# akanazawa/human_dynamics

Measured on NVIDIA H100. Metric: frames/sec (ResNet->f_movie->SMPL LBS), higher is better.
Workload: dtype f32 (wgmma 3x fp16 head/remainder split, fp32 two-level accumulate)

## Files before the change

### human_dynamics_b200/csrc/conv_tc.cu

```cuda
#include <cuda.h>
#include <cuda_fp16.h>
#include <cstdlib>
#include "conv_common.cuh"
#include "tc_ptx.cuh"

namespace hd {
namespace {

constexpr int BM = 128;
constexpr int A_TILE_BYTES = BM * 128;
constexpr int BOX_BYTES = 64 * 128;
constexpr int W_PROD = 8;
constexpr int STAGE_OUT = 1, STAGE_PAIR = 2;

using namespace ptx;

template <bool SPLIT, bool HALF, bool ASPLIT, int BN, bool RES = false, bool SHORT = false>
struct Cfg {
  static_assert(BN == 64 || (BN == 128 && HALF && ASPLIT), "128-wide N tiles: pre-split fp16 path only");
  static_assert(!RES || ASPLIT, "residual by TMA: pre-split fp16 path only");
  static_assert(!SHORT || (BN == 64 && HALF && ASPLIT), "two CTAs per SM: 64-wide pre-split fp16 tiles only");
  static constexpr int CTAS = SHORT ? 2 : 1;
  static constexpr int PROD_THREADS = BN == 128 || SHORT ? 128 : 256;
  static constexpr int NUM_THREADS = 256 + PROD_THREADS;
  static constexpr int ROW_STEP = PROD_THREADS / 8;
  static constexpr int ROWS = BM / ROW_STEP;
  static constexpr int PROD_REGS = SHORT ? 32 : BN == 128 ? 40 : 104, CONS_REGS = SHORT ? 104 : BN == 128 ? 232 : 152;
  static_assert(CTAS * (256 * CONS_REGS + PROD_THREADS * PROD_REGS) <= 65536, "setmaxnreg split beyond the register file");
  static constexpr int NACC = BN / 2;
  static constexpr int STAGES = SHORT ? 1 : BN == 128 ? (RES ? 2 : 3) : (RES ? 3 : 4);
  static constexpr int BKE = HALF ? 64 : 32;
  static constexpr int B_TILE_BYTES = BN * 128;
  static constexpr int B_OFFSET = (SPLIT ? 2 : 1) * A_TILE_BYTES;
  static constexpr int STAGE_BYTES = (SPLIT ? 2 : 1) * (A_TILE_BYTES + B_TILE_BYTES);
  static constexpr int RES_OFFSET = STAGES * STAGE_BYTES;
  static constexpr int RES_SLOT_BYTES = RES || SHORT ? 64 * BN * 4 : 0;
  static constexpr int STG_OFFSET = SHORT ? RES_OFFSET : RES_OFFSET + 2 * RES_SLOT_BYTES;
  static constexpr int STG_BYTES = ASPLIT ? 2 * BOX_BYTES : 0;
  static_assert(!SHORT || STG_BYTES == RES_SLOT_BYTES, "SHORT: the staging buffer is the residual slot");
  static constexpr int BAR_OFFSET = SHORT ? RES_OFFSET + 2 * RES_SLOT_BYTES : STG_OFFSET + 2 * STG_BYTES;
  static constexpr int SMEM_BYTES = BAR_OFFSET + 128 + 1024;
  static_assert(SMEM_BYTES <= 232448, "dynamic shared memory beyond the 227 KB a CTA can opt into");
  static_assert(CTAS * (SMEM_BYTES + 1024) <= 233472, "CTAS CTAs (and the 1 KB each reserves) beyond an SM's 228 KB");
  static constexpr int PF = HALF ? 2 : 3;
  static constexpr int V = HALF ? 2 : 1;
};

template <int R>
struct RowState {
  int n[R], iy[R], ix[R];
};

template <bool SPLIT, int PCH, bool HALF, bool GATHER, bool ASPLIT, int BN, bool RES, bool SHORT>
__global__ void __launch_bounds__((Cfg<SPLIT, HALF, ASPLIT, BN, RES, SHORT>::NUM_THREADS), (Cfg<SPLIT, HALF, ASPLIT, BN, RES, SHORT>::CTAS))
conv_gemm_tc_kernel(const ConvParams p, const __grid_constant__ CUtensorMap tmap_hi, const __grid_constant__ CUtensorMap tmap_lo,
                    const __grid_constant__ CUtensorMap tmap_res, const __grid_constant__ CUtensorMap tmap_out,
                    const __grid_constant__ CUtensorMap tmap_out_hi, const __grid_constant__ CUtensorMap tmap_out_lo, const int stage) {
  using C = Cfg<SPLIT, HALF, ASPLIT, BN, RES, SHORT>;
  constexpr bool MEM_STAMPS = BN == 128 || SHORT;
  constexpr int BKE = C::BKE, PF = C::PF, V = C::V, STAGES = C::STAGES, R = C::ROWS, RS = C::ROW_STEP, NA = C::NACC;
  extern __shared__ uint8_t smem_raw[];
  const uint32_t smem_base = (smem_u32(smem_raw) + 1023u) & ~1023u;
  uint8_t *smem = smem_raw + (smem_base - smem_u32(smem_raw));
  const uint32_t bar_base = smem_base + C::BAR_OFFSET;
  auto full_bar = [&](int s) { return bar_base + 8u * s; };
  auto empty_bar = [&](int s) { return bar_base + 8u * (STAGES + s); };
  auto res_bar = [&](int g) { return bar_base + 8u * (2 * STAGES + g); };

  const int warp = threadIdx.x >> 5, lane = threadIdx.x & 31;
  const int num_k = (GATHER ? p.K_pad : p.K) / BKE;
  const int tiles_n = (p.Cout + BN - 1) / BN;
  const int num_tiles = ((p.M + BM - 1) / BM) * tiles_n;
  const int my_tiles = (num_tiles - (int)blockIdx.x + (int)gridDim.x - 1) / (int)gridDim.x;

  if (threadIdx.x == 0) {
    for (int s = 0; s < STAGES; ++s) {
      mbar_init(full_bar(s), ASPLIT ? C::PROD_THREADS + 1 : 9);
      mbar_init(empty_bar(s), 8);
    }
    if (RES) for (int g = 0; g < 2; ++g) mbar_init(res_bar(g), 1);
    asm volatile("fence.mbarrier_init.release.cluster;" ::: "memory");
  }
  __syncthreads();

  if (warp >= W_PROD) {
    asm volatile("setmaxnreg.dec.sync.aligned.u32 %0;" ::"n"(C::PROD_REGS));
    const int t = threadIdx.x - W_PROD * 32;
    const int j = t & 7;
    const int rb = t >> 3;
    const uint32_t sw_off = (uint32_t)((j ^ (rb & 7)) << 4);
    const bool prof = p.dbg != nullptr && blockIdx.x == 0 && t == 0;
    long long t_wait = 0, t_start = prof && !MEM_STAMPS ? clock64() : 0;
    if (MEM_STAMPS && prof) { p.dbg[0] = clock64(); p.dbg[1] = 0; }
    auto wait_empty = [&](int s, uint32_t ph) {
      if (MEM_STAMPS && prof) p.dbg[1] -= clock64();
      const long long tw0 = !MEM_STAMPS && prof ? clock64() : 0;
      mbar_wait(empty_bar(s), ph ^ 1u);
      if (!MEM_STAMPS && prof) t_wait += clock64() - tw0;
      if (MEM_STAMPS && prof) p.dbg[1] += clock64();
    };
    const int total = my_tiles * num_k;
    auto load_b = [&](int s, int ti, int kc) {
      if (t != 0) return;
      const int n0 = (((int)blockIdx.x + ti * (int)gridDim.x) % tiles_n) * BN;
      const uint32_t b_hi = smem_base + s * C::STAGE_BYTES + C::B_OFFSET;
      const int boxes = (BN == 128 && n0 + 64 < p.Cout) ? 2 : 1;
      mbar_arrive_expect_tx(full_bar(s), (SPLIT ? 2 : 1) * boxes * BOX_BYTES);
      for (int b = 0; b < boxes; ++b) {
        tma_load_2d(b_hi + b * BOX_BYTES, &tmap_hi, full_bar(s), kc * BKE, n0 + 64 * b);
        if (SPLIT) tma_load_2d(b_hi + C::B_TILE_BYTES + b * BOX_BYTES, &tmap_lo, full_bar(s), kc * BKE, n0 + 64 * b);
      }
    };

    auto enter_tile = [&](int ti, RowState<R> &rs) {
      const int tile = (int)blockIdx.x + ti * (int)gridDim.x;
      const int m0 = (tile / tiles_n) * BM;
      const int hw = p.Ho * p.Wo;
#pragma unroll
      for (int i = 0; i < R; ++i) {
        const int m = m0 + rb + RS * i;
        if (m < p.M) {
          const int n = m / hw;
          const int r = m - n * hw;
          const int oy = r / p.Wo, ox = r - oy * p.Wo;
          rs.n[i] = n; rs.iy[i] = oy * p.stride - p.pad_t; rs.ix[i] = ox * p.stride - p.pad_l;
        } else {
          rs.n[i] = -1; rs.iy[i] = 0; rs.ix[i] = 0;
        }
      }
    };
    if constexpr (ASPLIT) {
      const __half *ihi = reinterpret_cast<const __half *>(p.in_hi);
      const __half *ilo = reinterpret_cast<const __half *>(p.in_lo);
      if (SHORT || (!p.planes && p.KH * p.KW <= 32 && (long long)p.n_img * p.H * p.W * p.in_ld < (1ll << 31))) {
        const uint32_t off0 = (uint32_t)rb * 128u + sw_off;
        int base[R];
        uint32_t mask[R];
        int kc = 0, ti = 0, tap = 0, ci0 = 0, kx = 0, ky = 0, tap_off = 0;
        for (int q = 0; q < total; ++q) {
          if (kc == 0) {
            const int tile = (int)blockIdx.x + ti * (int)gridDim.x;
            const int m0 = (tile / tiles_n) * BM + rb;
            const int hw = p.Ho * p.Wo;
#pragma unroll
            for (int i = 0; i < R; ++i) {
              const int m = m0 + RS * i;
              uint32_t mk = 0;
              int b = 0;
              if (m < p.M) {
                const int n = m / hw;
                const int r = m - n * hw;
                const int oy = r / p.Wo, ox = r - oy * p.Wo;
                const int iy0 = oy * p.stride - p.pad_t, ix0 = ox * p.stride - p.pad_l;
                b = ((n * p.H + iy0) * p.W + ix0) * p.in_ld + j * 8;
                int t = 0;
                for (int yy = 0; yy < p.KH; ++yy)
                  for (int xx = 0; xx < p.KW; ++xx, ++t)
                    if ((unsigned)(iy0 + yy) < (unsigned)p.H && (unsigned)(ix0 + xx) < (unsigned)p.W) mk |= 1u << t;
              }
              base[i] = SHORT && !(mk & 1u) ? -1 : b;
              mask[i] = mk;
            }
            tap = 0; ci0 = 0; kx = 0; ky = 0; tap_off = 0;
          }
          const int s = q % STAGES;
          const uint32_t ph = (uint32_t)(q / STAGES) & 1u;
          wait_empty(s, ph);
          load_b(s, ti, kc);
          const uint32_t a_hi = smem_base + s * C::STAGE_BYTES + off0;
          const int eo = SHORT ? ci0 : tap_off + ci0;
#pragma unroll
          for (int i = 0; i < R; ++i) {
            const bool ok = SHORT ? base[i] >= 0 : (mask[i] >> tap) & 1u;
            const int e = ok ? base[i] + eo : 0;
            cp_async16(a_hi + i * RS * 128, ihi + e, ok ? 16u : 0u);
            if (SPLIT) cp_async16(a_hi + A_TILE_BYTES + i * RS * 128, ilo + e, ok ? 16u : 0u);
          }
          asm volatile("cp.async.mbarrier.arrive.noinc.shared::cta.b64 [%0];" ::"r"(full_bar(s)) : "memory");
          ci0 += BKE;
          if (ci0 == p.Cin) {
            ci0 = 0; ++tap;
            if (++kx == p.KW) { kx = 0; ++ky; }
            tap_off = (ky * p.W + kx) * p.in_ld;
          }
          if (++kc == num_k) { kc = 0; ++ti; }
        }
      } else if (!SHORT && p.planes && (long long)p.n_img * p.H * p.W * p.in_ld < (1ll << 31)) {
        const uint32_t off0 = (uint32_t)rb * 128u + sw_off;
        const int jt = j >> 2;
        const int row_step = 2 * p.W * (int)p.in_ld;
        int base[R];
        int kc = 0, ti = 0;
        for (int q = 0; q < total; ++q) {
          if (kc == 0) {
            const int tile = (int)blockIdx.x + ti * (int)gridDim.x;
            const int m0 = (tile / tiles_n) * BM + rb;
            const int hw = p.Ho * p.Wo;
#pragma unroll
            for (int i = 0; i < R; ++i) {
              const int m = m0 + RS * i;
              int b = -1;
              if (m < p.M) {
                const int n = m / hw;
                const int r = m - n * hw;
                const int oy = r / p.Wo, ox = r - oy * p.Wo;
                b = ((n * p.H + oy * p.stride + jt) * p.W + ox * p.stride) * (int)p.in_ld + (j & 3) * 8;
              }
              base[i] = b;
            }
          }
          const int s = q % STAGES;
          const uint32_t ph = (uint32_t)(q / STAGES) & 1u;
          wait_empty(s, ph);
          load_b(s, ti, kc);
          const uint32_t a_hi = smem_base + s * C::STAGE_BYTES + off0;
          const bool tap_ok = 2 * kc + jt < 7;
          const int eo = kc * row_step;
#pragma unroll
          for (int i = 0; i < R; ++i) {
            const bool ok = tap_ok && base[i] >= 0;
            const int e = ok ? base[i] + eo : 0;
            cp_async16_ca(a_hi + i * RS * 128, ihi + e, ok ? 16u : 0u);
            if (SPLIT) cp_async16_ca(a_hi + A_TILE_BYTES + i * RS * 128, ilo + e, ok ? 16u : 0u);
          }
          asm volatile("cp.async.mbarrier.arrive.noinc.shared::cta.b64 [%0];" ::"r"(full_bar(s)) : "memory");
          if (++kc == num_k) { kc = 0; ++ti; }
        }
      } else if (!SHORT) {
      RowState<R> rs;
      int kc = 0, ti = 0;
      for (int q = 0; q < total; ++q) {
        if (kc == 0) enter_tile(ti, rs);
        const int s = q % STAGES;
        const uint32_t ph = (uint32_t)(q / STAGES) & 1u;
        wait_empty(s, ph);
        load_b(s, ti, kc);
        const int kb = kc * BKE;
        const int tap = p.planes ? 2 * kc + (j >> 2) : kb / p.Cin;
        const int ci = p.planes ? (j & 3) * 8 : kb - tap * p.Cin + j * 8;
        const int ky = tap / p.KW, kx = tap - ky * p.KW;
        const bool tap_ok = !p.planes || tap < 7;
        const uint32_t a_hi = smem_base + s * C::STAGE_BYTES, a_lo = a_hi + A_TILE_BYTES;
#pragma unroll
        for (int i = 0; i < R; ++i) {
          const int iy = rs.iy[i] + ky, ix = rs.ix[i] + kx;
          const bool ok = tap_ok && rs.n[i] >= 0 && iy >= 0 && iy < p.H && ix >= 0 && ix < p.W;
          const size_t e = ok ? ((size_t)((size_t)rs.n[i] * p.H + iy) * p.W + ix) * p.in_ld + ci : 0;
          const uint32_t off = (uint32_t)(rb + RS * i) * 128u + sw_off;
          if (p.planes) {
            cp_async16_ca(a_hi + off, ihi + e, ok ? 16u : 0u);
            if (SPLIT) cp_async16_ca(a_lo + off, ilo + e, ok ? 16u : 0u);
          } else {
            cp_async16(a_hi + off, ihi + e, ok ? 16u : 0u);
            if (SPLIT) cp_async16(a_lo + off, ilo + e, ok ? 16u : 0u);
          }
        }
        asm volatile("cp.async.mbarrier.arrive.noinc.shared::cta.b64 [%0];" ::"r"(full_bar(s)) : "memory");
        if (++kc == num_k) { kc = 0; ++ti; }
      }
      }
      cp_async_commit();
      cp_async_wait<0>();
      if (prof) { p.dbg[0] = clock64() - (MEM_STAMPS ? p.dbg[0] : t_start); if (!MEM_STAMPS) p.dbg[1] = t_wait; }
    } else {
    RowState<R> pf_rs, st_rs;
    float4 ring[PF][4 * V];
    uint32_t vmask[PF];
    int pf_kc = 0, pf_ti = 0;
    auto prefetch = [&](float4 *dst, uint32_t &vm) {
      if (pf_kc == 0) enter_tile(pf_ti, pf_rs);
      if (GATHER) {
        const int seg = p.KW * p.Cin, segp = (seg + 7) & ~7;
        const int g8 = (pf_kc * BKE + j * (4 * V)) / 8;
        const int gpr = segp >> 3;
        const int ky = g8 / gpr, r0 = (g8 - ky * gpr) * 8;
// ... 18 lines not shown
        if (++pf_kc == num_k) { pf_kc = 0; ++pf_ti; }
        return;
      }
      const int kb = pf_kc * BKE;
      const int tap = kb / p.Cin, ci = kb - tap * p.Cin + j * (4 * V);
      const int ky = tap / p.KW, kx = tap - ky * p.KW;
      vm = 0;
#pragma unroll
      for (int i = 0; i < 4; ++i) {
        const int iy = pf_rs.iy[i] + ky, ix = pf_rs.ix[i] + kx;
        const bool ok = pf_rs.n[i] >= 0 && (unsigned)iy < (unsigned)p.H && (unsigned)ix < (unsigned)p.W;
        if (ok) {
          const float4 *src = reinterpret_cast<const float4 *>(p.in + ((size_t)((size_t)pf_rs.n[i] * p.H + iy) * p.W + ix) * p.in_ld + ci);
#pragma unroll
          for (int v = 0; v < V; ++v) dst[i * V + v] = __ldg(src + v);
          vm |= 1u << i;
        } else {
#pragma unroll
          for (int v = 0; v < V; ++v) dst[i * V + v] = make_float4(0.f, 0.f, 0.f, 0.f);
        }
      }
      if (++pf_kc == num_k) { pf_kc = 0; ++pf_ti; }
    };
    int st_kc = 0, st_ti = 0;
    auto consume = [&](int q, float4 *cur, uint32_t vm) {
      if (st_kc == 0) enter_tile(st_ti, st_rs);
      const int s = q % STAGES;
      const uint32_t ph = (uint32_t)(q / STAGES) & 1u;
      long long tw0 = prof ? clock64() : 0;
      mbar_wait(empty_bar(s), ph ^ 1u);
      if (prof) t_wait += clock64() - tw0;
      load_b(s, st_ti, st_kc);
      uint8_t *a_hi = smem + s * C::STAGE_BYTES;
      uint8_t *a_lo = a_hi + A_TILE_BYTES;
      const int pci = p.pre_scale ? (st_kc * BKE) % p.Cin + j * (4 * V) : 0;
#pragma unroll
      for (int i = 0; i < 4; ++i) {
        float xs[4 * V];
#pragma unroll
        for (int v = 0; v < V; ++v) {
          const float4 x = cur[i * V + v];
          xs[4 * v] = x.x; xs[4 * v + 1] = x.y; xs[4 * v + 2] = x.z; xs[4 * v + 3] = x.w;
        }
        if (p.pre_scale && (vm & (1u << i))) {
          const size_t po = (size_t)(p.pre_img_stride != 0 ? st_rs.n[i] : 0) * p.pre_img_stride + pci;
#pragma unroll
          for (int v = 0; v < V; ++v) {
            const float4 sc = __ldg(reinterpret_cast<const float4 *>(p.pre_scale + po) + v);
            const float4 sh = __ldg(reinterpret_cast<const float4 *>(p.pre_shift + po) + v);
            xs[4 * v] = xs[4 * v] * sc.x + sh.x; xs[4 * v + 1] = xs[4 * v + 1] * sc.y + sh.y;
            xs[4 * v + 2] = xs[4 * v + 2] * sc.z + sh.z; xs[4 * v + 3] = xs[4 * v + 3] * sc.w + sh.w;
          }
          if (p.pre_relu) {
#pragma unroll
            for (int e = 0; e < 4 * V; ++e) xs[e] = fmaxf(xs[e], 0.f);
          }
        }
        uint32_t h[4], l[4];
        if (!HALF) {
#pragma unroll
          for (int e = 0; e < 4; ++e) {
            const float hf = rn_tf32(xs[e]);
            h[e] = __float_as_uint(hf);
            l[e] = __float_as_uint(rn_tf32(xs[e] - hf));
          }
        } else {
#pragma unroll
// ... 39 lines not shown
    for (int i = 0; i < NA; ++i) {
      acc[i] = 0.f;
      if constexpr (SPLIT) accx[i] = 0.f;
    }
    uint8_t *res_sm = smem + C::RES_OFFSET + wg * C::RES_SLOT_BYTES;
    const bool res_issuer = RES && (threadIdx.x & 127) == 0;
    const bool stg_issuer = ASPLIT && (threadIdx.x & 127) == 0;
    auto load_res = [&](int ti) {
      const int tile = (int)blockIdx.x + ti * (int)gridDim.x;
      const int r0 = (tile / tiles_n) * BM + 64 * wg, c0 = (tile % tiles_n) * BN;
      const int cols = p.Cout - c0 < BN ? p.Cout - c0 : BN;
      const int boxes = r0 < p.M ? (cols + 31) / 32 : 0;
      const uint32_t slot = smem_base + C::RES_OFFSET + wg * C::RES_SLOT_BYTES;
      mbar_arrive_expect_tx(res_bar(wg), boxes * (64 * 128));
      for (int b = 0; b < boxes; ++b) tma_load_2d(slot + b * (64 * 128), &tmap_res, res_bar(wg), c0 + 32 * b, r0);
    };
    if (res_issuer && my_tiles > 0) load_res(0);
    int q = 0;
    for (int ti = 0; ti < my_tiles; ++ti) {
      if (!SHORT) {
#pragma unroll
        for (int i = 0; i < NA; ++i) sums[i] = 0.f;
      }
      for (int kc = 0; kc < num_k; ++kc, ++q) {
        const int s = q % STAGES;
        const uint32_t ph = (uint32_t)(q / STAGES) & 1u;
        const bool group_start = (kc % PCH) == 0;
        if (MEM_STAMPS && prof) p.dbg[3] -= clock64();
        const long long tw0 = !MEM_STAMPS && prof ? clock64() : 0;
        mbar_wait(full_bar(s), ph);
        if (!MEM_STAMPS && prof) t_wait += clock64() - tw0;
        if (MEM_STAMPS && prof) p.dbg[3] += clock64();
        if (ASPLIT) asm volatile("fence.proxy.async.shared::cta;" ::: "memory");
        const uint32_t a_hi = smem_base + s * C::STAGE_BYTES + wg * (64 * 128);
        const uint32_t a_lo = a_hi + A_TILE_BYTES;
        const uint32_t b_hi = smem_base + s * C::STAGE_BYTES + C::B_OFFSET;
        const uint32_t b_lo = b_hi + C::B_TILE_BYTES;
        const uint64_t da_hi = make_smem_desc(a_hi), da_lo = make_smem_desc(a_lo);
        const uint64_t db_hi = make_smem_desc(b_hi), db_lo = make_smem_desc(b_lo);
        fence_regs(acc);
        if constexpr (SPLIT) fence_regs(accx);
        wgmma_fence();
#pragma unroll
        for (int k = 0; k < 4; ++k) {
          const uint64_t adv = (uint64_t)((k * 32) >> 4);
          if constexpr (BN == 128) {
            if constexpr (SPLIT) {
              wgmma_m64n128k16_f16(accx, da_lo + adv, db_hi + adv, (kc | k) != 0);
              wgmma_m64n128k16_f16(accx, da_hi + adv, db_lo + adv, 1u);
            }
            wgmma_m64n128k16_f16(acc, da_hi + adv, db_hi + adv, !(group_start && k == 0));
          } else if constexpr (HALF) {
            if constexpr (SPLIT) {
              wgmma_m64n64k16_f16(accx, da_lo + adv, db_hi + adv, (kc | k) != 0);
              wgmma_m64n64k16_f16(accx, da_hi + adv, db_lo + adv, 1u);
            }
            wgmma_m64n64k16_f16(acc, da_hi + adv, db_hi + adv, !(group_start && k == 0));
          } else {
            if constexpr (SPLIT) {
              wgmma_m64n64k8_tf32(accx, da_lo + adv, db_hi + adv, (kc | k) != 0);
              wgmma_m64n64k8_tf32(accx, da_hi + adv, db_lo + adv, 1u);
            }
            wgmma_m64n64k8_tf32(acc, da_hi + adv, db_hi + adv, !(group_start && k == 0));
          }
        }
        wgmma_commit();
        wgmma_wait<0>();
        fence_regs(acc);
        if constexpr (SPLIT) fence_regs(accx);
        __syncwarp();
        if (lane == 0) mbar_arrive(empty_bar(s));
        if (!SHORT && ((kc % PCH) == PCH - 1 || kc == num_k - 1)) {
#pragma unroll
          for (int i = 0; i < NA; ++i) sums[i] += acc[i];
        }
      }
      if (SHORT) {
#pragma unroll
        for (int i = 0; i < NA; ++i) acc[i] = __fadd_rn(0.f, acc[i]);
      }
      if constexpr (SPLIT) {
#pragma unroll
        for (int i = 0; i < NA; ++i) sums[i] += accx[i] * (HALF ? (1.0f / 2048.0f) : 1.0f);
      }
      if (prof) p.dbg[4] -= clock64();
      const int tile = (int)blockIdx.x + ti * (int)gridDim.x;
      const int m0 = (tile / tiles_n) * BM, n0 = (tile % tiles_n) * BN;
      if (RES && prof) p.dbg[5] -= clock64();
      if (RES) mbar_wait(res_bar(wg), (uint32_t)ti & 1u);
      if (RES && prof) p.dbg[5] += clock64();
      auto row_geom = [&](int m, int &n_img, int &oy, int &ox) {
        n_img = 0; oy = 0; ox = 0;
        if (p.out_sub || (!RES && p.res && !(p.res_stride == 1 && p.res_H == p.Ho && p.res_W == p.Wo))) {
          n_img = m / hw;
          const int r = m - n_img * hw;
          oy = r / p.Wo; ox = r - oy * p.Wo;
        }
      };
      auto res_row = [&](int m, int n_img, int oy, int ox) -> const float * {
        if (RES || !p.res) return nullptr;
        const size_t rr = (p.res_stride == 1 && p.res_H == p.Ho && p.res_W == p.Wo)
                              ? (size_t)m
                              : ((size_t)n_img * p.res_H + (size_t)oy * p.res_stride) * p.res_W + (size_t)ox * p.res_stride;
        return p.res + rr * p.res_ld;
      };
      auto out_row = [&](int m, int n_img, int oy, int ox) -> float * {
        if (!p.out) return nullptr;
        if (!p.out_sub) return p.out + (size_t)m * p.out_ld;
        if (oy % p.out_sub != 0 || ox % p.out_sub != 0) return nullptr;
        const int Hs = (p.Ho + p.out_sub - 1) / p.out_sub, Ws = (p.Wo + p.out_sub - 1) / p.out_sub;
        return p.out + ((size_t)((size_t)n_img * Hs + oy / p.out_sub) * Ws + ox / p.out_sub) * p.out_ld;
      };
      auto value2 = [&](int c, const float2 *rs, const float *rrow, float &y0, float &y1) {
        if (p.post_scale) { const float2 sc = __ldg(reinterpret_cast<const float2 *>(p.post_scale + c)); y0 *= sc.x; y1 *= sc.y; }
        if (p.post_shift) { const float2 sh = __ldg(reinterpret_cast<const float2 *>(p.post_shift + c)); y0 += sh.x; y1 += sh.y; }
        if (RES) { const float2 r = *rs; y0 += r.x; y1 += r.y; }
        else if (rrow) { const float2 r = *reinterpret_cast<const float2 *>(rrow + c); y0 += r.x; y1 += r.y; }
        if (p.post_relu) { y0 = fmaxf(y0, 0.f); y1 = fmaxf(y1, 0.f); }
      };
      auto pair2 = [&](int c, float a0, float a1, uint32_t &hh, uint32_t &ll) {
        if (p.post2_scale) { const float2 sc = __ldg(reinterpret_cast<const float2 *>(p.post2_scale + c)); a0 *= sc.x; a1 *= sc.y; }
        if (p.post2_shift) { const float2 sh = __ldg(reinterpret_cast<const float2 *>(p.post2_shift + c)); a0 += sh.x; a1 += sh.y; }
        if (p.post2_relu) { a0 = fmaxf(a0, 0.f); a1 = fmaxf(a1, 0.f); }
        split_f16x2(a0, a1, hh, ll);
      };
      if constexpr (ASPLIT) {
        const bool st32 = (stage & STAGE_OUT) != 0, st2 = (stage & STAGE_PAIR) != 0;
        uint8_t *stg = smem + C::STG_OFFSET + wg * C::STG_BYTES;
        const uint32_t stg_a = smem_base + C::STG_OFFSET + wg * C::STG_BYTES;
        const int r0 = m0 + 64 * wg;
        const uint32_t rsw = (uint32_t)(lane >> 2);
        auto acquire = [&](bool after_out) {
          if (prof) p.dbg[6] -= clock64();
          if (stg_issuer) {
            if (after_out) bulk_wait_read<1>();
            else bulk_wait_read<0>();
          }
          named_bar_sync(3 + wg, 128);
          if (prof) p.dbg[6] += clock64();
        };
#pragma unroll
        for (int cc = 0; cc < BN / 64; ++cc) {
          const int c0 = n0 + 64 * cc;
          const bool issue = stg_issuer && r0 < p.M && c0 < p.Cout;
          if (st32 && !RES) acquire(false);
          const bool rok[2] = {m0 + frow < p.M, m0 + frow + 8 < p.M};
          if (st32 && (RES || !p.res)) {
            uint8_t *brow = (RES ? res_sm + 2 * cc * BOX_BYTES : stg) + (frow - 64 * wg) * 128 + 8 * (lane & 1);
            const float *vsc = p.post_scale ? p.post_scale + c0 + fcol : nullptr, *vsh = p.post_shift ? p.post_shift + c0 + fcol : nullptr;
#pragma unroll
            for (int jj = 0; jj < 8; ++jj) {
              const int j = 8 * cc + jj;
              if (c0 + 8 * jj + fcol >= p.Cout) continue;
              const uint32_t piece = (uint32_t)(2 * (jj & 3) + ((lane & 3) >> 1)) ^ rsw;
              const float2 sc = vsc ? __ldg(reinterpret_cast<const float2 *>(vsc + 8 * jj)) : make_float2(0.f, 0.f);
              const float2 sh = vsh ? __ldg(reinterpret_cast<const float2 *>(vsh + 8 * jj)) : make_float2(0.f, 0.f);
#pragma unroll
              for (int h = 0; h < 2; ++h) {
                if (!rok[h]) continue;
                float2 *f32 = reinterpret_cast<float2 *>(brow + h * 1024 + (jj >> 2) * BOX_BYTES + piece * 16);
                float y0 = sums[4 * j + 2 * h], y1 = sums[4 * j + 2 * h + 1];
                if (vsc) { y0 = __fmul_rn(y0, sc.x); y1 = __fmul_rn(y1, sc.y); }
                if (vsh) { y0 = __fadd_rn(y0, sh.x); y1 = __fadd_rn(y1, sh.y); }
                if (RES) { const float2 r = *f32; y0 = __fadd_rn(y0, r.x); y1 = __fadd_rn(y1, r.y); }
                if (p.post_relu) { y0 = fmaxf(y0, 0.f); y1 = fmaxf(y1, 0.f); }
                *f32 = make_float2(y0, y1);
                sums[4 * j + 2 * h] = y0; sums[4 * j + 2 * h + 1] = y1;
              }
            }
          } else {
#pragma unroll
          for (int h = 0; h < 2; ++h) {
            const int m = m0 + frow + 8 * h;
            if (m >= p.M) continue;
            int n_img, oy, ox;
            row_geom(m, n_img, oy, ox);
            const float *rrow = res_row(m, n_img, oy, ox);
            float *orow = st32 ? nullptr : out_row(m, n_img, oy, ox);
            uint8_t *brow = (RES ? res_sm + 2 * cc * BOX_BYTES : stg) + (frow - 64 * wg + 8 * h) * 128 + 8 * (lane & 1);
// ... 113 lines not shown
          } else {
#pragma unroll
            for (int e = 0; e < 2; ++e) {
              if (e == 1 && !two) break;
              float v = y[e];
              if (p.post_scale) v *= __ldg(p.post_scale + c + e);
              if (p.post_shift) v += __ldg(p.post_shift + c + e);
              if (rrow) v += rrow[c + e];
              if (p.post_relu) v = fmaxf(v, 0.f);
              if (orow) orow[c + e] = v;
            }
          }
        }
      }
      }
      if (RES && ti + 1 < my_tiles) {
        if (prof) p.dbg[6] -= clock64();
        named_bar_sync(1 + wg, 128);
        if (res_issuer) {
          if (SHORT) {
            if (stage) bulk_wait_read<0>();
          } else if (stage & STAGE_OUT) {
            if (stage & STAGE_PAIR) bulk_wait_read<1>();
            else bulk_wait_read<0>();
          }
          load_res(ti + 1);
        }
        if (prof) p.dbg[6] += clock64();
      }
      if (prof) p.dbg[4] += clock64();
    }
    if (stg_issuer) bulk_wait_all();
    if (prof) { p.dbg[2] = clock64() - (RES || MEM_STAMPS ? p.dbg[2] : t_start); if (!MEM_STAMPS) p.dbg[3] = t_wait; }
  }
}

typedef CUresult (*EncodeTiledFn)(CUtensorMap *, CUtensorMapDataType, cuuint32_t, void *, const cuuint64_t *, const cuuint64_t *,
                                  const cuuint32_t *, const cuuint32_t *, CUtensorMapInterleave, CUtensorMapSwizzle,
                                  CUtensorMapL2promotion, CUtensorMapFloatOOBfill);

EncodeTiledFn get_encode_fn() {
  static EncodeTiledFn fn = nullptr;
  static bool tried = false;
  if (!tried) {
    tried = true;
    void *ptr = nullptr;
    cudaDriverEntryPointQueryResult qres;
    cudaError_t e = cudaGetDriverEntryPoint("cuTensorMapEncodeTiled", &ptr, cudaEnableDefault, &qres);
    if (e == cudaSuccess && qres == cudaDriverEntryPointSuccess) fn = reinterpret_cast<EncodeTiledFn>(ptr);
    else (void)cudaGetLastError();
  }
  return fn;
}

constexpr int kMaxDevices = 64;

int encode_epilogue_map(CUtensorMap *tm, bool fp16, const void *base, int cols, int rows, long long ld_bytes, const char *what) {
  EncodeTiledFn fn = get_encode_fn();
  if (!fn) { set_last_error_text("cuTensorMapEncodeTiled unavailable (no CUDA driver?)"); return HD_ERR_UNSUPPORTED; }
  const cuuint64_t gdim[2] = {(cuuint64_t)cols, (cuuint64_t)rows};
  const cuuint64_t gstride[1] = {(cuuint64_t)ld_bytes};
  const cuuint32_t box[2] = {fp16 ? 64u : 32u, 64u};
  const cuuint32_t estr[2] = {1u, 1u};
  CUresult r = fn(tm, fp16 ? CU_TENSOR_MAP_DATA_TYPE_FLOAT16 : CU_TENSOR_MAP_DATA_TYPE_FLOAT32, 2, const_cast<void *>(base), gdim, gstride,
                  box, estr, CU_TENSOR_MAP_INTERLEAVE_NONE, CU_TENSOR_MAP_SWIZZLE_128B, CU_TENSOR_MAP_L2_PROMOTION_L2_128B,
                  CU_TENSOR_MAP_FLOAT_OOB_FILL_NONE);
  if (r != CUDA_SUCCESS) {
    char msg[96];
    snprintf(msg, sizeof(msg), "cuTensorMapEncodeTiled (%s) failed with CUresult %d", what, (int)r);
    set_last_error_text(msg);
    return HD_ERR_CUDA;
  }
  return HD_OK;
}

template <bool SPLIT, int PCH, bool HALF, bool GATHER = false, bool ASPLIT = false, int BN = 64, bool RES = false, bool SHORT = false>
int launch_tc(const ConvParams &p, const hd_conv_desc *d, cudaStream_t st) {
  using C = Cfg<SPLIT, HALF, ASPLIT, BN, RES, SHORT>;
  static bool configured[kMaxDevices] = {};
  static int num_sms[kMaxDevices] = {};
  int dev = 0;
  cudaGetDevice(&dev);
  if (dev < 0 || dev >= kMaxDevices) { set_last_error_text("conv_gemm_tc: device ordinal out of range"); return HD_ERR_UNSUPPORTED; }
  if (!configured[dev]) {
    cudaError_t e = cudaFuncSetAttribute(conv_gemm_tc_kernel<SPLIT, PCH, HALF, GATHER, ASPLIT, BN, RES, SHORT>,
                                         cudaFuncAttributeMaxDynamicSharedMemorySize, C::SMEM_BYTES);
    if (e != cudaSuccess) { set_last_error("conv_gemm_tc attr", e); return HD_ERR_CUDA; }
    cudaDeviceGetAttribute(&num_sms[dev], cudaDevAttrMultiProcessorCount, dev);
    if (num_sms[dev] <= 0) { set_last_error_text("conv_gemm_tc: no multiprocessor count"); return HD_ERR_CUDA; }
    configured[dev] = true;
  }
  alignas(64) CUtensorMap thi, tlo;
  const void *mhi = d->tmap_hi_n64 ? d->tmap_hi_n64 : d->tmap_hi;
  const void *mlo = d->tmap_hi_n64 ? d->tmap_lo_n64 : d->tmap_lo;
  memcpy(&thi, mhi, sizeof(CUtensorMap));
  memcpy(&tlo, mlo ? mlo : mhi, sizeof(CUtensorMap));
  alignas(64) CUtensorMap tres, tout, tohi, tolo;
  memcpy(&tres, &thi, sizeof(CUtensorMap));
  memcpy(&tout, &thi, sizeof(CUtensorMap));
  memcpy(&tohi, &thi, sizeof(CUtensorMap));
  memcpy(&tolo, &thi, sizeof(CUtensorMap));
  int rc = HD_OK;
  if (RES) rc = encode_epilogue_map(&tres, false, p.res, p.Cout, p.M, p.res_ld * 4, "residual");
  int stage = 0;
  if (ASPLIT && p.out && !p.out_sub) {
    stage |= STAGE_OUT;
    if (rc == HD_OK) rc = encode_epilogue_map(&tout, false, p.out, p.Cout, p.M, p.out_ld * 4, "output");
  }
  if (ASPLIT && p.out_hi && p.out2_ld % 8 == 0) {
    stage |= STAGE_PAIR;
    if (rc == HD_OK) rc = encode_epilogue_map(&tohi, true, p.out_hi, p.Cout, p.M, p.out2_ld * 2, "output head");
    if (rc == HD_OK && SPLIT) rc = encode_epilogue_map(&tolo, true, p.out_lo, p.Cout, p.M, p.out2_ld * 2, "output remainder");
  }
  if (rc != HD_OK) return rc;
  const int num_tiles = ceil_div(p.M, BM) * ceil_div(p.Cout, BN);
  const int ctas = C::CTAS * num_sms[dev];
  dim3 grid(num_tiles < ctas ? num_tiles : ctas);
  conv_gemm_tc_kernel<SPLIT, PCH, HALF, GATHER, ASPLIT, BN, RES, SHORT>
      <<<grid, C::NUM_THREADS, C::SMEM_BYTES, st>>>(p, thi, tlo, tres, tout, tohi, tolo, stage);
  return check_launch("conv_gemm_tc_kernel");
}

bool wide_n_tile(const ConvParams &p) {
  if (p.Cout <= 64) return false;
  int dev = 0, sms = 0;
  cudaGetDevice(&dev);
  cudaDeviceGetAttribute(&sms, cudaDevAttrMultiProcessorCount, dev);
  if (sms <= 0) return true;
  const long long m_tiles = ceil_div(p.M, BM);
  const long long w128 = (m_tiles * ceil_div(p.Cout, 128) + sms - 1) / sms, w64 = (m_tiles * ceil_div(p.Cout, 64) + sms - 1) / sms;
  return 16 * w128 <= 9 * w64;
}

template <bool SPLIT, bool RES>
bool short_k_two_ctas() {
  using C = Cfg<SPLIT, true, true, 64, RES, true>;
  static int two[kMaxDevices] = {};
  int dev = 0;
  cudaGetDevice(&dev);
  if (dev < 0 || dev >= kMaxDevices) return false;
  if (two[dev] == 0) {
    const auto kernel = conv_gemm_tc_kernel<SPLIT, 2, true, false, true, 64, RES, true>;
    int n = 0;
    if (cudaFuncSetAttribute(kernel, cudaFuncAttributeMaxDynamicSharedMemorySize, C::SMEM_BYTES) != cudaSuccess ||
        cudaOccupancyMaxActiveBlocksPerMultiprocessor(&n, kernel, C::NUM_THREADS, C::SMEM_BYTES) != cudaSuccess) {
      (void)cudaGetLastError();
      n = 0;
    }
    two[dev] = n >= 2 ? 1 : -1;
  }
  return two[dev] > 0;
}

template <bool SPLIT>
int launch_conv_f16(const ConvParams &p, const hd_conv_desc *d, cudaStream_t st) {
  if (p.in_hi && p.planes) {
    if (p.Cin != 32 || p.KH != 8 || p.KW != 1 || p.stride != 2 || p.pad_t != 0 || p.pad_l != 0 || p.in_ld != 4 || p.Cout > 64 ||
        p.W % 2 != 0 || 2 * (p.Wo - 1) + 8 > p.W || 2 * (p.Ho - 1) + 7 > p.H || !aligned16(p.in_hi) || !aligned16(p.in_lo) || p.pre_scale) {
      set_last_error_text("hd_conv_gemm(tc planes): needs the conv1 plane geometry (Cin 32, KH 8, KW 1, stride 2, in_ld 4, even W)");
      return HD_ERR_INVALID;
    }
    return launch_tc<SPLIT, 2, true, false, true>(p, d, st);
  }
  if (p.in_hi) {
    if (p.Cin % 64 != 0 || p.K % 64 != 0 || p.in_ld % 8 != 0 || !aligned16(p.in_hi) || !aligned16(p.in_lo) || p.pre_scale) {
      set_last_error_text("hd_conv_gemm(tc split-A): needs Cin % 64 == 0, in_ld % 8 == 0, aligned in_hi/in_lo, no prologue");
      return HD_ERR_INVALID;
    }
    const bool res_rows = p.res && p.res_stride == 1 && p.res_H == p.Ho && p.res_W == p.Wo && p.K <= 8 * 64;
    const bool short_k = p.K <= 2 * 64 && p.KH * p.KW == 1 && (long long)p.n_img * p.H * p.W * p.in_ld < (1ll << 31) &&
                         (p.res ? res_rows : p.out_hi != nullptr);
    if (short_k && (res_rows ? short_k_two_ctas<SPLIT, true>() : short_k_two_ctas<SPLIT, false>()))
      return res_rows ? launch_tc<SPLIT, 2, true, false, true, 64, true, true>(p, d, st)
                      : launch_tc<SPLIT, 2, true, false, true, 64, false, true>(p, d, st);
    if (wide_n_tile(p))
      return res_rows ? launch_tc<SPLIT, 2, true, false, true, 128, true>(p, d, st) : launch_tc<SPLIT, 2, true, false, true, 128>(p, d, st);
    return res_rows ? launch_tc<SPLIT, 2, true, false, true, 64, true>(p, d, st) : launch_tc<SPLIT, 2, true, false, true>(p, d, st);
  }
  if (p.Cin % 64 != 0) {
    const int segp = (p.KW * p.Cin + 7) & ~7;
    if (p.K_pad % 64 != 0 || p.K_pad < p.KH * segp || p.Cout > 64 || p.pre_scale || p.in_ld != p.Cin) {
      set_last_error_text("hd_conv_gemm(tc gather): needs K_pad % 64 == 0, K_pad >= KH*roundup8(KW*Cin), Cout <= 64, dense pixels, no prologue");
      return HD_ERR_INVALID;
    }
    return launch_tc<SPLIT, 2, true, true>(p, d, st);
  }
  if (!p.in || p.in_ld % 4 != 0 || !aligned16(p.in) || p.K % 64 != 0 ||
      (p.pre_scale && (!aligned16(p.pre_scale) || !aligned16(p.pre_shift) || p.pre_img_stride % 4 != 0))) {
    set_last_error_text("hd_conv_gemm(tc): needs Cin % 32 (tf32) / % 64 (fp16) == 0 and 16-byte aligned input / prologue vectors");
    return HD_ERR_INVALID;
  }
  return launch_tc<SPLIT, 2, true>(p, d, st);
}

}
// ... 80 lines not shown
```

Baseline: 13200.

## Add channels-on-M wgmma variant for conv1 planes with 256-row pixel tiles

Adds a CM configuration for the conv1 plane path (Cout 64) in which the weight tile serves as the wgmma M operand and a 256-pixel tile serves as N, using m64n128k16 per warpgroup. Each CTA now covers twice as many output rows with two pipeline stages and a transposed fp32 epilogue that writes through TMA. The variant is chosen only when the tile count per SM drops enough. A separate fused fp16 pair-only epilogue path is also added for the non-residual ASPLIT case. The trade-off is fewer stages, higher register pressure, and a more complex swizzled transposed store.

New measurement: 13650, median of 6. 1.03x the previous value.

```diff
diff --git a/human_dynamics_b200/csrc/conv_tc.cu b/human_dynamics_b200/csrc/conv_tc.cu
--- a/human_dynamics_b200/csrc/conv_tc.cu
+++ b/human_dynamics_b200/csrc/conv_tc.cu
@@ -8,35 +8,38 @@
 namespace {
 
 constexpr int BM = 128;
-constexpr int A_TILE_BYTES = BM * 128;
 constexpr int BOX_BYTES = 64 * 128;
 constexpr int W_PROD = 8;
 constexpr int STAGE_OUT = 1, STAGE_PAIR = 2;
 
 using namespace ptx;
 
-template <bool SPLIT, bool HALF, bool ASPLIT, int BN, bool RES = false, bool SHORT = false>
+template <bool SPLIT, bool HALF, bool ASPLIT, int BN, bool RES = false, bool SHORT = false, bool CM = false>
 struct Cfg {
   static_assert(BN == 64 || (BN == 128 && HALF && ASPLIT), "128-wide N tiles: pre-split fp16 path only");
   static_assert(!RES || ASPLIT, "residual by TMA: pre-split fp16 path only");
   static_assert(!SHORT || (BN == 64 && HALF && ASPLIT), "two CTAs per SM: 64-wide pre-split fp16 tiles only");
+  static_assert(!CM || (BN == 64 && HALF && ASPLIT && !RES && !SHORT), "channels on M: 64-channel pre-split fp16 tiles, no residual");
   static constexpr int CTAS = SHORT ? 2 : 1;
-  static constexpr int PROD_THREADS = BN == 128 || SHORT ? 128 : 256;
+  static constexpr int TM = CM ? 256 : BM;
+  static constexpr int A_BYTES = TM * 128;
+  static constexpr int PROD_THREADS = BN == 128 || SHORT || CM ? 128 : 256;
   static constexpr int NUM_THREADS = 256 + PROD_THREADS;
   static constexpr int ROW_STEP = PROD_THREADS / 8;
-  static constexpr int ROWS = BM / ROW_STEP;
-  static constexpr int PROD_REGS = SHORT ? 32 : BN == 128 ? 40 : 104, CONS_REGS = SHORT ? 104 : BN == 128 ? 232 : 152;
-  static_assert(CTAS * (256 * CONS_REGS + PROD_THREADS * PROD_REGS) <= 65536, "setmaxnreg split beyond the register file");
-  static constexpr int NACC = BN / 2;
-  static constexpr int STAGES = SHORT ? 1 : BN == 128 ? (RES ? 2 : 3) : (RES ? 3 : 4);
+  static constexpr int ROWS = TM / ROW_STEP;
+  static constexpr int PROD_REGS = SHORT ? 32 : CM ? 56 : BN == 128 ? 40 : 104, CONS_REGS = SHORT ? 104 : CM ? 224 : BN == 128 ? 232 : 152;
+  static_assert(256 * CONS_REGS + PROD_THREADS * PROD_REGS <= NUM_THREADS * (65536 / (CTAS * NUM_THREADS) / 8 * 8),
+                "setmaxnreg split beyond the CTA's registers");
+  static constexpr int NACC = CM ? 64 : BN / 2;
+  static constexpr int STAGES = SHORT ? 1 : CM ? 2 : BN == 128 ? (RES ? 2 : 3) : (RES ? 3 : 4);
   static constexpr int BKE = HALF ? 64 : 32;
   static constexpr int B_TILE_BYTES = BN * 128;
-  static constexpr int B_OFFSET = (SPLIT ? 2 : 1) * A_TILE_BYTES;
-  static constexpr int STAGE_BYTES = (SPLIT ? 2 : 1) * (A_TILE_BYTES + B_TILE_BYTES);
+  static constexpr int B_OFFSET = (SPLIT ? 2 : 1) * A_BYTES;
+  static constexpr int STAGE_BYTES = (SPLIT ? 2 : 1) * (A_BYTES + B_TILE_BYTES);
   static constexpr int RES_OFFSET = STAGES * STAGE_BYTES;
   static constexpr int RES_SLOT_BYTES = RES || SHORT ? 64 * BN * 4 : 0;
   static constexpr int STG_OFFSET = SHORT ? RES_OFFSET : RES_OFFSET + 2 * RES_SLOT_BYTES;
-  static constexpr int STG_BYTES = ASPLIT ? 2 * BOX_BYTES : 0;
+  static constexpr int STG_BYTES = ASPLIT ? (CM ? 4 : 2) * BOX_BYTES : 0;
   static_assert(!SHORT || STG_BYTES == RES_SLOT_BYTES, "SHORT: the staging buffer is the residual slot");
   static constexpr int BAR_OFFSET = SHORT ? RES_OFFSET + 2 * RES_SLOT_BYTES : STG_OFFSET + 2 * STG_BYTES;
   static constexpr int SMEM_BYTES = BAR_OFFSET + 128 + 1024;
@@ -51,13 +54,13 @@
   int n[R], iy[R], ix[R];
 };
 
-template <bool SPLIT, int PCH, bool HALF, bool GATHER, bool ASPLIT, int BN, bool RES, bool SHORT>
-__global__ void __launch_bounds__((Cfg<SPLIT, HALF, ASPLIT, BN, RES, SHORT>::NUM_THREADS), (Cfg<SPLIT, HALF, ASPLIT, BN, RES, SHORT>::CTAS))
+template <bool SPLIT, int PCH, bool HALF, bool GATHER, bool ASPLIT, int BN, bool RES, bool SHORT, bool CM>
+__global__ void __launch_bounds__((Cfg<SPLIT, HALF, ASPLIT, BN, RES, SHORT, CM>::NUM_THREADS), (Cfg<SPLIT, HALF, ASPLIT, BN, RES, SHORT, CM>::CTAS))
 conv_gemm_tc_kernel(const ConvParams p, const __grid_constant__ CUtensorMap tmap_hi, const __grid_constant__ CUtensorMap tmap_lo,
                     const __grid_constant__ CUtensorMap tmap_res, const __grid_constant__ CUtensorMap tmap_out,
                     const __grid_constant__ CUtensorMap tmap_out_hi, const __grid_constant__ CUtensorMap tmap_out_lo, const int stage) {
-  using C = Cfg<SPLIT, HALF, ASPLIT, BN, RES, SHORT>;
-  constexpr bool MEM_STAMPS = BN == 128 || SHORT;
+  using C = Cfg<SPLIT, HALF, ASPLIT, BN, RES, SHORT, CM>;
+  constexpr bool MEM_STAMPS = BN == 128 || SHORT || CM;
   constexpr int BKE = C::BKE, PF = C::PF, V = C::V, STAGES = C::STAGES, R = C::ROWS, RS = C::ROW_STEP, NA = C::NACC;
   extern __shared__ uint8_t smem_raw[];
   const uint32_t smem_base = (smem_u32(smem_raw) + 1023u) & ~1023u;
@@ -70,7 +73,7 @@
   const int warp = threadIdx.x >> 5, lane = threadIdx.x & 31;
   const int num_k = (GATHER ? p.K_pad : p.K) / BKE;
   const int tiles_n = (p.Cout + BN - 1) / BN;
-  const int num_tiles = ((p.M + BM - 1) / BM) * tiles_n;
+  const int num_tiles = ((p.M + C::TM - 1) / C::TM) * tiles_n;
   const int my_tiles = (num_tiles - (int)blockIdx.x + (int)gridDim.x - 1) / (int)gridDim.x;
 
   if (threadIdx.x == 0) {
@@ -114,7 +117,7 @@
 
     auto enter_tile = [&](int ti, RowState<R> &rs) {
       const int tile = (int)blockIdx.x + ti * (int)gridDim.x;
-      const int m0 = (tile / tiles_n) * BM;
+      const int m0 = (tile / tiles_n) * C::TM;
       const int hw = p.Ho * p.Wo;
 #pragma unroll
       for (int i = 0; i < R; ++i) {
@@ -132,7 +135,7 @@
     if constexpr (ASPLIT) {
       const __half *ihi = reinterpret_cast<const __half *>(p.in_hi);
       const __half *ilo = reinterpret_cast<const __half *>(p.in_lo);
-      if (SHORT || (!p.planes && p.KH * p.KW <= 32 && (long long)p.n_img * p.H * p.W * p.in_ld < (1ll << 31))) {
+      if (SHORT || (!CM && !p.planes && p.KH * p.KW <= 32 && (long long)p.n_img * p.H * p.W * p.in_ld < (1ll << 31))) {
         const uint32_t off0 = (uint32_t)rb * 128u + sw_off;
         int base[R];
         uint32_t mask[R];
@@ -140,7 +143,7 @@
         for (int q = 0; q < total; ++q) {
           if (kc == 0) {
             const int tile = (int)blockIdx.x + ti * (int)gridDim.x;
-            const int m0 = (tile / tiles_n) * BM + rb;
+            const int m0 = (tile / tiles_n) * C::TM + rb;
             const int hw = p.Ho * p.Wo;
 #pragma unroll
             for (int i = 0; i < R; ++i) {
@@ -174,7 +177,7 @@
             const bool ok = SHORT ? base[i] >= 0 : (mask[i] >> tap) & 1u;
             const int e = ok ? base[i] + eo : 0;
             cp_async16(a_hi + i * RS * 128, ihi + e, ok ? 16u : 0u);
-            if (SPLIT) cp_async16(a_hi + A_TILE_BYTES + i * RS * 128, ilo + e, ok ? 16u : 0u);
+            if (SPLIT) cp_async16(a_hi + C::A_BYTES + i * RS * 128, ilo + e, ok ? 16u : 0u);
           }
           asm volatile("cp.async.mbarrier.arrive.noinc.shared::cta.b64 [%0];" ::"r"(full_bar(s)) : "memory");
           ci0 += BKE;
@@ -194,7 +197,7 @@
         for (int q = 0; q < total; ++q) {
           if (kc == 0) {
             const int tile = (int)blockIdx.x + ti * (int)gridDim.x;
-            const int m0 = (tile / tiles_n) * BM + rb;
+            const int m0 = (tile / tiles_n) * C::TM + rb;
             const int hw = p.Ho * p.Wo;
 #pragma unroll
             for (int i = 0; i < R; ++i) {
@@ -221,12 +224,12 @@
             const bool ok = tap_ok && base[i] >= 0;
             const int e = ok ? base[i] + eo : 0;
             cp_async16_ca(a_hi + i * RS * 128, ihi + e, ok ? 16u : 0u);
-            if (SPLIT) cp_async16_ca(a_hi + A_TILE_BYTES + i * RS * 128, ilo + e, ok ? 16u : 0u);
+            if (SPLIT) cp_async16_ca(a_hi + C::A_BYTES + i * RS * 128, ilo + e, ok ? 16u : 0u);
           }
           asm volatile("cp.async.mbarrier.arrive.noinc.shared::cta.b64 [%0];" ::"r"(full_bar(s)) : "memory");
           if (++kc == num_k) { kc = 0; ++ti; }
         }
-      } else if (!SHORT) {
+      } else if (!SHORT && !CM) {
       RowState<R> rs;
       int kc = 0, ti = 0;
       for (int q = 0; q < total; ++q) {
@@ -240,7 +243,7 @@
         const int ci = p.planes ? (j & 3) * 8 : kb - tap * p.Cin + j * 8;
         const int ky = tap / p.KW, kx = tap - ky * p.KW;
         const bool tap_ok = !p.planes || tap < 7;
-        const uint32_t a_hi = smem_base + s * C::STAGE_BYTES, a_lo = a_hi + A_TILE_BYTES;
+        const uint32_t a_hi = smem_base + s * C::STAGE_BYTES, a_lo = a_hi + C::A_BYTES;
 #pragma unroll
         for (int i = 0; i < R; ++i) {
           const int iy = rs.iy[i] + ky, ix = rs.ix[i] + kx;
@@ -325,7 +328,7 @@
       if (prof) t_wait += clock64() - tw0;
       load_b(s, st_ti, st_kc);
       uint8_t *a_hi = smem + s * C::STAGE_BYTES;
-      uint8_t *a_lo = a_hi + A_TILE_BYTES;
+      uint8_t *a_lo = a_hi + C::A_BYTES;
       const int pci = p.pre_scale ? (st_kc * BKE) % p.Cin + j * (4 * V) : 0;
 #pragma unroll
       for (int i = 0; i < 4; ++i) {
@@ -431,8 +434,8 @@
         if (!MEM_STAMPS && prof) t_wait += clock64() - tw0;
         if (MEM_STAMPS && prof) p.dbg[3] += clock64();
         if (ASPLIT) asm volatile("fence.proxy.async.shared::cta;" ::: "memory");
-        const uint32_t a_hi = smem_base + s * C::STAGE_BYTES + wg * (64 * 128);
-        const uint32_t a_lo = a_hi + A_TILE_BYTES;
+        const uint32_t a_hi = smem_base + s * C::STAGE_BYTES + wg * (C::TM / 2 * 128);
+        const uint32_t a_lo = a_hi + C::A_BYTES;
         const uint32_t b_hi = smem_base + s * C::STAGE_BYTES + C::B_OFFSET;
         const uint32_t b_lo = b_hi + C::B_TILE_BYTES;
         const uint64_t da_hi = make_smem_desc(a_hi), da_lo = make_smem_desc(a_lo);
@@ -443,7 +446,13 @@
 #pragma unroll
         for (int k = 0; k < 4; ++k) {
           const uint64_t adv = (uint64_t)((k * 32) >> 4);
-          if constexpr (BN == 128) {
+          if constexpr (CM) {
+            if constexpr (SPLIT) {
+              wgmma_m64n128k16_f16(accx, db_hi + adv, da_lo + adv, (kc | k) != 0);
+              wgmma_m64n128k16_f16(accx, db_lo + adv, da_hi + adv, 1u);
+            }
+            wgmma_m64n128k16_f16(acc, db_hi + adv, da_hi + adv, !(group_start && k == 0));
+          } else if constexpr (BN == 128) {
             if constexpr (SPLIT) {
               wgmma_m64n128k16_f16(accx, da_lo + adv, db_hi + adv, (kc | k) != 0);
               wgmma_m64n128k16_f16(accx, da_hi + adv, db_lo + adv, 1u);
@@ -484,7 +493,7 @@
       }
       if (prof) p.dbg[4] -= clock64();
       const int tile = (int)blockIdx.x + ti * (int)gridDim.x;
-      const int m0 = (tile / tiles_n) * BM, n0 = (tile % tiles_n) * BN;
+      const int m0 = (tile / tiles_n) * C::TM, n0 = (tile % tiles_n) * BN;
       if (RES && prof) p.dbg[5] -= clock64();
       if (RES) mbar_wait(res_bar(wg), (uint32_t)ti & 1u);
       if (RES && prof) p.dbg[5] += clock64();
@@ -523,7 +532,49 @@
         if (p.post2_relu) { a0 = fmaxf(a0, 0.f); a1 = fmaxf(a1, 0.f); }
         split_f16x2(a0, a1, hh, ll);
       };
-      if constexpr (ASPLIT) {
+      if constexpr (CM) {
+        const bool st32 = (stage & STAGE_OUT) != 0;
+        uint8_t *stg = smem + C::STG_OFFSET + wg * C::STG_BYTES;
+        const uint32_t stg_a = smem_base + C::STG_OFFSET + wg * C::STG_BYTES;
+        const int r0 = m0 + 128 * wg;
+        const int ch = (warp & 3) * 16 + (lane >> 2);
+        auto acquire = [&]() {
+          if (prof) p.dbg[6] -= clock64();
+          if (stg_issuer) bulk_wait_read<0>();
+          named_bar_sync(3 + wg, 128);
+          if (prof) p.dbg[6] += clock64();
+        };
+        if (st32) {
+          acquire();
+#pragma unroll
+          for (int h = 0; h < 2; ++h) {
+            const int c = ch + 8 * h;
+            const float sc = p.post_scale ? __ldg(p.post_scale + c) : 0.f, sh = p.post_shift ? __ldg(p.post_shift + c) : 0.f;
+            uint8_t *cb = stg + (c >> 5) * BOX_BYTES + (c & 3) * 4;
+#pragma unroll
+            for (int j = 0; j < 16; ++j) {
+#pragma unroll
+              for (int e = 0; e < 2; ++e) {
+                const int r = 8 * (j & 7) + fcol + e;
+                float y = sums[4 * j + 2 * h + e];
+                if (p.post_scale) y = __fmul_rn(y, sc);
+                if (p.post_shift) y = __fadd_rn(y, sh);
+                if (p.post_relu) y = fmaxf(y, 0.f);
+                *reinterpret_cast<float *>(cb + (j >> 3) * 2 * BOX_BYTES + r * 128 + ((((c & 31) >> 2) ^ (fcol + e)) << 4)) = y;
+                sums[4 * j + 2 * h + e] = y;
+              }
+            }
+          }
+          fence_proxy_async();
+          named_bar_sync(3 + wg, 128);
+          if (stg_issuer) {
+#pragma unroll
+            for (int b = 0; b < 4; ++b)
+              if (r0 + 64 * (b >> 1) < p.M) tma_store_2d(&tmap_out, stg_a + b * BOX_BYTES, 32 * (b & 1), r0 + 64 * (b >> 1));
+            bulk_commit();
+          }
+        }
+      } else if constexpr (ASPLIT) {
         const bool st32 = (stage & STAGE_OUT) != 0, st2 = (stage & STAGE_PAIR) != 0;
         uint8_t *stg = smem + C::STG_OFFSET + wg * C::STG_BYTES;
         const uint32_t stg_a = smem_base + C::STG_OFFSET + wg * C::STG_BYTES;
@@ -544,6 +595,45 @@
           const bool issue = stg_issuer && r0 < p.M && c0 < p.Cout;
           if (st32 && !RES) acquire(false);
           const bool rok[2] = {m0 + frow < p.M, m0 + frow + 8 < p.M};
+          if (!RES && !st32 && st2 && !p.out && !p.res) {
+            acquire(false);
+            uint8_t *brow = stg + (frow - 64 * wg) * 128 + 4 * (lane & 3);
+            const float *vsc = p.post_scale ? p.post_scale + c0 + fcol : nullptr, *vsh = p.post_shift ? p.post_shift + c0 + fcol : nullptr;
+            const float *v2sc = p.post2_scale ? p.post2_scale + c0 + fcol : nullptr, *v2sh = p.post2_shift ? p.post2_shift + c0 + fcol : nullptr;
+#pragma unroll
+            for (int jj = 0; jj < 8; ++jj) {
+              const int j = 8 * cc + jj;
+              if (c0 + 8 * jj + fcol >= p.Cout) continue;
+              const float2 sc = vsc ? __ldg(reinterpret_cast<const float2 *>(vsc + 8 * jj)) : make_float2(0.f, 0.f);
+              const float2 sh = vsh ? __ldg(reinterpret_cast<const float2 *>(vsh + 8 * jj)) : make_float2(0.f, 0.f);
+              const float2 sc2 = v2sc ? __ldg(reinterpret_cast<const float2 *>(v2sc + 8 * jj)) : make_float2(0.f, 0.f);
+              const float2 sh2 = v2sh ? __ldg(reinterpret_cast<const float2 *>(v2sh + 8 * jj)) : make_float2(0.f, 0.f);
+#pragma unroll
+              for (int h = 0; h < 2; ++h) {
+                if (!rok[h]) continue;
+                float a0 = sums[4 * j + 2 * h], a1 = sums[4 * j + 2 * h + 1];
+                if (vsc) { a0 = __fmul_rn(a0, sc.x); a1 = __fmul_rn(a1, sc.y); }
+                if (vsh) { a0 = __fadd_rn(a0, sh.x); a1 = __fadd_rn(a1, sh.y); }
+                if (p.post_relu) { a0 = fmaxf(a0, 0.f); a1 = fmaxf(a1, 0.f); }
+                if (v2sc) { a0 = __fmul_rn(a0, sc2.x); a1 = __fmul_rn(a1, sc2.y); }
+                if (v2sh) { a0 = __fadd_rn(a0, sh2.x); a1 = __fadd_rn(a1, sh2.y); }
+                if (p.post2_relu) { a0 = fmaxf(a0, 0.f); a1 = fmaxf(a1, 0.f); }
+                uint32_t hh, ll;
+                split_f16x2(a0, a1, hh, ll);
+                uint32_t *hs = reinterpret_cast<uint32_t *>(brow + h * 1024 + (((uint32_t)jj ^ rsw) * 16));
+                hs[0] = hh;
+                if (SPLIT) hs[BOX_BYTES / 4] = ll;
+              }
+            }
+            fence_proxy_async();
+            named_bar_sync(3 + wg, 128);
+            if (issue) {
+              tma_store_2d(&tmap_out_hi, stg_a, c0, r0);
+              if (SPLIT) tma_store_2d(&tmap_out_lo, stg_a + BOX_BYTES, c0, r0);
+            }
+            if (stg_issuer) bulk_commit();
+            continue;
+          }
           if (st32 && (RES || !p.res)) {
             uint8_t *brow = (RES ? res_sm + 2 * cc * BOX_BYTES : stg) + (frow - 64 * wg) * 128 + 8 * (lane & 1);
             const float *vsc = p.post_scale ? p.post_scale + c0 + fcol : nullptr, *vsh = p.post_shift ? p.post_shift + c0 + fcol : nullptr;
@@ -723,6 +813,7 @@
     }
     if (stg_issuer) bulk_wait_all();
     if (prof) { p.dbg[2] = clock64() - (RES || MEM_STAMPS ? p.dbg[2] : t_start); if (!MEM_STAMPS) p.dbg[3] = t_wait; }
+    if (prof) { p.dbg[7] = C::TM; p.dbg[8] = BN; }
   }
 }
 
@@ -765,16 +856,17 @@
   return HD_OK;
 }
 
-template <bool SPLIT, int PCH, bool HALF, bool GATHER = false, bool ASPLIT = false, int BN = 64, bool RES = false, bool SHORT = false>
+template <bool SPLIT, int PCH, bool HALF, bool GATHER = false, bool ASPLIT = false, int BN = 64, bool RES = false, bool SHORT = false,
+          bool CM = false>
 int launch_tc(const ConvParams &p, const hd_conv_desc *d, cudaStream_t st) {
-  using C = Cfg<SPLIT, HALF, ASPLIT, BN, RES, SHORT>;
+  using C = Cfg<SPLIT, HALF, ASPLIT, BN, RES, SHORT, CM>;
   static bool configured[kMaxDevices] = {};
   static int num_sms[kMaxDevices] = {};
   int dev = 0;
   cudaGetDevice(&dev);
   if (dev < 0 || dev >= kMaxDevices) { set_last_error_text("conv_gemm_tc: device ordinal out of range"); return HD_ERR_UNSUPPORTED; }
   if (!configured[dev]) {
-    cudaError_t e = cudaFuncSetAttribute(conv_gemm_tc_kernel<SPLIT, PCH, HALF, GATHER, ASPLIT, BN, RES, SHORT>,
+    cudaError_t e = cudaFuncSetAttribute(conv_gemm_tc_kernel<SPLIT, PCH, HALF, GATHER, ASPLIT, BN, RES, SHORT, CM>,
                                          cudaFuncAttributeMaxDynamicSharedMemorySize, C::SMEM_BYTES);
     if (e != cudaSuccess) { set_last_error("conv_gemm_tc attr", e); return HD_ERR_CUDA; }
     cudaDeviceGetAttribute(&num_sms[dev], cudaDevAttrMultiProcessorCount, dev);
@@ -804,10 +896,10 @@
     if (rc == HD_OK && SPLIT) rc = encode_epilogue_map(&tolo, true, p.out_lo, p.Cout, p.M, p.out2_ld * 2, "output remainder");
   }
   if (rc != HD_OK) return rc;
-  const int num_tiles = ceil_div(p.M, BM) * ceil_div(p.Cout, BN);
+  const int num_tiles = ceil_div(p.M, C::TM) * ceil_div(p.Cout, BN);
   const int ctas = C::CTAS * num_sms[dev];
   dim3 grid(num_tiles < ctas ? num_tiles : ctas);
-  conv_gemm_tc_kernel<SPLIT, PCH, HALF, GATHER, ASPLIT, BN, RES, SHORT>
+  conv_gemm_tc_kernel<SPLIT, PCH, HALF, GATHER, ASPLIT, BN, RES, SHORT, CM>
       <<<grid, C::NUM_THREADS, C::SMEM_BYTES, st>>>(p, thi, tlo, tres, tout, tohi, tolo, stage);
   return check_launch("conv_gemm_tc_kernel");
 }
@@ -823,6 +915,18 @@
   return 16 * w128 <= 9 * w64;
 }
 
+
+bool cout_on_m(const ConvParams &p) {
+  if (!p.planes || p.Cout != 64 || p.res || p.out_sub || p.out_hi || !p.out) return false;
+  if ((long long)p.n_img * p.H * p.W * p.in_ld >= (1ll << 31)) return false;
+  int dev = 0, sms = 0;
+  cudaGetDevice(&dev);
+  cudaDeviceGetAttribute(&sms, cudaDevAttrMultiProcessorCount, dev);
+  if (sms <= 0) return true;
+  const long long w256 = (ceil_div(p.M, 256) + sms - 1) / sms, w128 = (ceil_div(p.M, BM) + sms - 1) / sms;
+  return 16 * w256 <= 9 * w128;
+}
+
 template <bool SPLIT, bool RES>
 bool short_k_two_ctas() {
   using C = Cfg<SPLIT, true, true, 64, RES, true>;
@@ -831,7 +935,7 @@
   cudaGetDevice(&dev);
   if (dev < 0 || dev >= kMaxDevices) return false;
   if (two[dev] == 0) {
-    const auto kernel = conv_gemm_tc_kernel<SPLIT, 2, true, false, true, 64, RES, true>;
+    const auto kernel = conv_gemm_tc_kernel<SPLIT, 2, true, false, true, 64, RES, true, false>;
     int n = 0;
     if (cudaFuncSetAttribute(kernel, cudaFuncAttributeMaxDynamicSharedMemorySize, C::SMEM_BYTES) != cudaSuccess ||
         cudaOccupancyMaxActiveBlocksPerMultiprocessor(&n, kernel, C::NUM_THREADS, C::SMEM_BYTES) != cudaSuccess) {
@@ -851,7 +955,7 @@
       set_last_error_text("hd_conv_gemm(tc planes): needs the conv1 plane geometry (Cin 32, KH 8, KW 1, stride 2, in_ld 4, even W)");
       return HD_ERR_INVALID;
     }
-    return launch_tc<SPLIT, 2, true, false, true>(p, d, st);
+    return cout_on_m(p) ? launch_tc<SPLIT, 2, true, false, true, 64, false, false, true>(p, d, st) : launch_tc<SPLIT, 2, true, false, true>(p, d, st);
   }
   if (p.in_hi) {
     if (p.Cin % 64 != 0 || p.K % 64 != 0 || p.in_ld % 8 != 0 || !aligned16(p.in_hi) || !aligned16(p.in_lo) || p.pre_scale) {
```
